# kakaobrain/rq-vae-transformer

Hardware: AMD Instinct MI355X
Metric: 256x256 images/sec, AR sampling + decode (RQ-Transformer huge, 8x8x4 codes) (higher is better)
Workload: dtype bf16

## Files before the change

### rq-vae-transformer_amd/csrc/rqt_kernels.hip

```cpp
#include "rqt_kernels.h"
#include "rq_common.h"
#include <mutex>
#include <stdlib.h>

static __device__ __forceinline__ float rq_u01(uint32_t r) { return fmaf((float)(r >> 9), 1.0f / 8388608.0f, 1.0f / 16777216.0f); }

#if defined(RQ_SAMPLE_GUIDED_TU) || defined(RQ_SAMPLE_ROWS_TU) || defined(RQ_SAMPLE_LOGP_TU)
#define RQ_SAMPLE_ONLY_TU 1
#endif
#ifndef RQ_SAMPLE_ONLY_TU

template <int NS>
__global__ __launch_bounds__(256) void resid_ln_kernel(ResidLnArgs p) {
    __shared__ float red[8];
    const int row = blockIdx.x, tid = threadIdx.x, lane = tid & 63, wave = tid >> 6;
    const int E = p.E, E4 = E >> 2;
    const long base = (long)row * E;
    const long slab_stride = (long)p.rows * E;
    f32x4 v[4];
#pragma unroll
    for (int i = 0; i < 4; ++i) {
        const int q = tid + 256 * i;
        v[i] = (f32x4){0.f, 0.f, 0.f, 0.f};
        if (q < E4) v[i] = *(const f32x4*)(p.x_in + base + q * 4);
// ... 902 lines not shown
        const int i = i0 + lane;
        const bool live = i < P;
        const int iq = live ? i : P - 1;
        float qf[64], acc[64];
#pragma unroll
        for (int c = 0; c < 8; ++c) unpack8(ld128(q0 + (long)iq * 3 * E + c * 8), qf + c * 8);
#pragma unroll
        for (int e = 0; e < 64; ++e) acc[e] = 0.f;
        float m = NEG_INF, l = 0.f;
        const int jend = i0 + 63 < P - 1 ? i0 + 63 : P - 1;
        for (int j = 0; j <= jend; ++j) {
            float dot = 0.f;
#pragma unroll
            for (int c = 0; c < 8; ++c) {
                float kf[8];
                unpack8(ld128(sK + j * 64 + c * 8), kf);
#pragma unroll
                for (int e = 0; e < 8; ++e) dot = fmaf(qf[c * 8 + e], kf[e], dot);
            }
            const float sc = j <= iq ? dot * 0.125f : NEG_INF;
            const float mn = fmaxf(m, sc);
            const float alpha = (m == NEG_INF) ? 0.f : rq_fast_exp2((m - mn) * 1.4426950408889634f);
            const float w = (sc == NEG_INF) ? 0.f : rq_fast_exp2((sc - mn) * 1.4426950408889634f);
            l = l * alpha + w;
            m = mn;
#pragma unroll
            for (int c = 0; c < 8; ++c) {
                float vf[8];
                unpack8(ld128(sV + j * 64 + c * 8), vf);
#pragma unroll
                for (int e = 0; e < 8; ++e) acc[c * 8 + e] = fmaf(w, vf[e], acc[c * 8 + e] * alpha);
            }
        }
        if (live) {
            const float inv = 1.0f / l;
            bf16_t* o = p.y + ((long)img * P + i) * E + hh * 64;
#pragma unroll
            for (int c = 0; c < 8; ++c) {
                rq_u128 u;
                u.x = pack_bf16x2(acc[c * 8 + 0] * inv, acc[c * 8 + 1] * inv); u.y = pack_bf16x2(acc[c * 8 + 2] * inv, acc[c * 8 + 3] * inv);
                u.z = pack_bf16x2(acc[c * 8 + 4] * inv, acc[c * 8 + 5] * inv); u.w = pack_bf16x2(acc[c * 8 + 6] * inv, acc[c * 8 + 7] * inv);
                st128(o + c * 8, u);
            }
        }
    }
}

#define ATTN_TILE_KEYS 64
template <bool APPEND>
__global__ __launch_bounds__(64) void attn_prefill_tiled_kernel(AttnPrefillArgs p) {
    constexpr int KT = ATTN_TILE_KEYS;
    __shared__ rq_u128 sK[KT * 8], sV[KT * 8];
    const int lane = threadIdx.x;
    const int P = p.P, E = p.E;
    const int nqt = (P + 63) / 64;
    const long blk = blockIdx.x;
    const int qt = nqt - 1 - (int)(blk % nqt);
    const long pair = blk / nqt;
    const int img = (int)(pair / p.nh), hh = (int)(pair - (long)img * p.nh);
    const bf16_t* q0 = p.qkv + (long)img * P * 3 * E + hh * 64;
    const int i0 = qt * 64, i = i0 + lane;
    const bool live = i < P;
    const int iq = live ? i : P - 1;
    const float NEG_INF = -__int_as_float(0x7f800000);
    float qf[64], acc[64];
#pragma unroll
    for (int c = 0; c < 8; ++c) unpack8(ld128(q0 + (long)iq * 3 * E + c * 8), qf + c * 8);
#pragma unroll
    for (int e = 0; e < 64; ++e) acc[e] = 0.f;
    float m = NEG_INF, l = 0.f;
    const int jend = i0 + 63 < P - 1 ? i0 + 63 : P - 1;
    for (int j0 = 0; j0 <= jend; j0 += KT) {
        const int nk = jend + 1 - j0 < KT ? jend + 1 - j0 : KT;
        rq_syncthreads();
        for (int idx = lane; idx < nk * 8; idx += 64) {
            const int j = j0 + (idx >> 3), c = idx & 7;
            const rq_u128 kv = ld128(q0 + (long)j * 3 * E + E + c * 8), vv = ld128(q0 + (long)j * 3 * E + 2 * E + c * 8);
            sK[idx] = kv;
            sV[idx] = vv;
            if (APPEND && j >= i0) {
                st128(p.kc + (pair * p.Tcap + j) * 64 + c * 8, kv);
                st128(p.vc + (pair * p.Tcap + j) * 64 + c * 8, vv);
            }
        }
        rq_syncthreads();
        for (int jj = 0; jj < nk; ++jj) {
            const int j = j0 + jj;
            float dot = 0.f;
#pragma unroll
            for (int c = 0; c < 8; ++c) {
                float kf[8];
                unpack8(sK[jj * 8 + c], kf);
#pragma unroll
                for (int e = 0; e < 8; ++e) dot = fmaf(qf[c * 8 + e], kf[e], dot);
            }
            const float sc = j <= iq ? dot * 0.125f : NEG_INF;
            const float mn = fmaxf(m, sc);
            const float alpha = (m == NEG_INF) ? 0.f : rq_fast_exp2((m - mn) * 1.4426950408889634f);
            const float w = (sc == NEG_INF) ? 0.f : rq_fast_exp2((sc - mn) * 1.4426950408889634f);
            l = l * alpha + w;
            m = mn;
#pragma unroll
            for (int c = 0; c < 8; ++c) {
                float vf[8];
                unpack8(sV[jj * 8 + c], vf);
#pragma unroll
                for (int e = 0; e < 8; ++e) acc[c * 8 + e] = fmaf(w, vf[e], acc[c * 8 + e] * alpha);
            }
        }
    }
    if (live) {
        const float inv = 1.0f / l;
        bf16_t* o = p.y + ((long)img * P + i) * E + hh * 64;
#pragma unroll
        for (int c = 0; c < 8; ++c) {
            rq_u128 u;
            u.x = pack_bf16x2(acc[c * 8 + 0] * inv, acc[c * 8 + 1] * inv); u.y = pack_bf16x2(acc[c * 8 + 2] * inv, acc[c * 8 + 3] * inv);
            u.z = pack_bf16x2(acc[c * 8 + 4] * inv, acc[c * 8 + 5] * inv); u.w = pack_bf16x2(acc[c * 8 + 6] * inv, acc[c * 8 + 7] * inv);
            st128(o + c * 8, u);
        }
    }
}

int rq_launch_attn_prefill(const AttnPrefillArgs& a, hipStream_t s) {
    const bool append = a.kc != nullptr;
    if (!append && (a.vc || a.ksc || a.vsc)) return rq_fail(RQAMD_ERR_INVALID, "prefill attention: cache-free form with a cache pointer");
    if (append && !a.vc) return rq_fail(RQAMD_ERR_INVALID, "prefill attention: key cache without a value cache");
    if (a.nh >= 1 && a.E != a.nh * 64) {
        RQ_TRY(attn_generic_check(a.E, a.nh, a.Tcap, a.ksc));
        if (a.P < 1 || a.P > a.Tcap) return rq_fail(RQAMD_ERR_UNSUPPORTED, "prefill attention: %d tokens (cache %d)", a.P, a.Tcap);
        const long blocks = (long)a.n_img * a.nh * a.P;
        if (blocks > 0x7fffffffL) return rq_fail(RQAMD_ERR_UNSUPPORTED, "prefill attention: %ld (image, head, token) triples", blocks);
        if (append) RQ_LAUNCH(attn_generic_prefill_kernel<true>, dim3((unsigned)blocks), dim3(64), 0, s, a);
        else RQ_LAUNCH(attn_generic_prefill_kernel<false>, dim3((unsigned)blocks), dim3(64), 0, s, a);
        return rq_check_launch("attn_generic_prefill_kernel");
    }
    if (a.nh < 1 || a.P < 1 || a.P > a.Tcap) return rq_fail(RQAMD_ERR_UNSUPPORTED, "prefill attention: %d tokens (cache %d)", a.P, a.Tcap);
    const char* force_tiled = getenv("RQAMD_PREFILL_TILED");
    if (a.P > 255 || (force_tiled && atoi(force_tiled) != 0 && !a.ksc)) {
        if (a.ksc || a.vsc) return rq_fail(RQAMD_ERR_UNSUPPORTED, "prefill attention: the 8-bit cache formats (RQAMD_KV) end at 255 prefix tokens (%d)", a.P);
        const long blocks = (long)a.n_img * a.nh * ((a.P + 63) / 64);
        if (blocks > 0x7fffffffL) return rq_fail(RQAMD_ERR_UNSUPPORTED, "prefill attention: %ld (image, head, query tile) triples", blocks);
        if (append) RQ_LAUNCH(attn_prefill_tiled_kernel<true>, dim3((unsigned)blocks), dim3(64), 0, s, a);
        else RQ_LAUNCH(attn_prefill_tiled_kernel<false>, dim3((unsigned)blocks), dim3(64), 0, s, a);
        return rq_check_launch("attn_prefill_tiled_kernel");
    }
    const size_t smem = (size_t)a.P * 64 * 2 * 2;
    if (append) RQ_LAUNCH(attn_prefill_kernel<true>, dim3((unsigned)(a.n_img * a.nh)), dim3(64), smem, s, a);
    else RQ_LAUNCH(attn_prefill_kernel<false>, dim3((unsigned)(a.n_img * a.nh)), dim3(64), smem, s, a);
    return rq_check_launch("attn_prefill_kernel");
}

__global__ void embed_tokens_kernel(EmbedTokArgs p) {
    const int per_row = p.dim / 8;
    const long gid = (long)blockIdx.x * blockDim.x + threadIdx.x;
    if (gid >= (long)p.rows * per_row) return;
    const int b = (int)(gid / per_row), c = (int)(gid - (long)b * per_row);
    const int pos = (p.pos ? *p.pos : 0) + p.pos_off;
    const int64_t* codes = p.xs + ((long)b * p.HW + pos) * p.D;
    float acc[8];
#pragma unroll
    for (int e = 0; e < 8; ++e) acc[e] = 0.f;
    for (int d = p.depth_lo; d < p.n_depth; ++d) {
        long code = codes[d];
        if (code < 0 || code >= p.K[d]) continue;
        const float* src = p.cb[d] + code * p.dim + c * 8;
        f32x4 a = *(const f32x4*)src, bq = *(const f32x4*)(src + 4);
#pragma unroll
        for (int e = 0; e < 4; ++e) { acc[e] += a[e]; acc[4 + e] += bq[e]; }
    }
    rq_u128 o;
    o.x = pack_bf16x2(acc[0], acc[1]); o.y = pack_bf16x2(acc[2], acc[3]);
    o.z = pack_bf16x2(acc[4], acc[5]); o.w = pack_bf16x2(acc[6], acc[7]);
    st128(p.out + (long)b * p.dim + c * 8, o);
}

int rq_launch_embed_tokens(const EmbedTokArgs& a, hipStream_t s) {
    if (a.dim % 8 != 0) return rq_fail(RQAMD_ERR_UNSUPPORTED, "embed: dim %d %% 8 != 0", a.dim);
    const long n = (long)a.rows * (a.dim / 8);
    RQ_LAUNCH(embed_tokens_kernel, dim3((unsigned)((n + 255) / 256)), dim3(256), 0, s, a);
    return rq_check_launch("embed_tokens_kernel");
}

__global__ void tok_embed_kernel(TokEmbedArgs p) {
    const int per_row = p.E / 4;
    const long gid = (long)blockIdx.x * blockDim.x + threadIdx.x;
    if (gid >= (long)p.rows * per_row) return;
    const int b = (int)(gid / per_row), c = (int)(gid - (long)b * per_row);
    const int pv = p.pos ? *p.pos : 0;
    const int64_t* codes = p.xs + ((long)b * p.HW + pv + p.pos_off) * p.D;
    const int arow = (p.add_by_pos ? pv : 0) + p.add_row;
    f32x4 acc = *(const f32x4*)(p.add + (long)arow * p.E + c * 4);
    for (int d = p.d_lo; d < p.d_hi; ++d) {
        long code = codes[d];
        if (code < 0 || code >= p.V[d]) rq_trap();
        acc = acc + *(const f32x4*)(p.table + ((long)p.offs[d] + code) * p.E + c * 4);
    }
    *(f32x4*)(p.out + (long)b * p.E + c * 4) = acc;
}
int rq_launch_tok_embed(const TokEmbedArgs& a, hipStream_t s) {
    const long n = (long)a.rows * (a.E / 4);
    RQ_LAUNCH(tok_embed_kernel, dim3((unsigned)((n + 255) / 256)), dim3(256), 0, s, a);
    return rq_check_launch("tok_embed_kernel");
}
__global__ void mask_logits_kernel(float* logits, int rows, int V, int v_lo) {
    const int w = V - v_lo;
    const long gid = (long)blockIdx.x * blockDim.x + threadIdx.x;
    if (gid >= (long)rows * w) return;
    const int r = (int)(gid / w), c = (int)(gid - (long)r * w);
    logits[(long)r * V + v_lo + c] = -__int_as_float(0x7f800000);
}
int rq_launch_mask_logits(float* logits, int rows, int V, int v_lo, hipStream_t s) {
    if (v_lo >= V) return RQAMD_OK;
    const long n = (long)rows * (V - v_lo);
    RQ_LAUNCH(mask_logits_kernel, dim3((unsigned)((n + 255) / 256)), dim3(256), 0, s, logits, rows, V, v_lo);
    return rq_check_launch("mask_logits_kernel");
}

__global__ void cond_embed_kernel(const int64_t* cond, int cond_stride, int cond_idx, const float* cond_emb, int vocab_cond,
                                  const float* pos_emb_cond, float* x, int rows, int E) {
    const long gid = (long)blockIdx.x * blockDim.x + threadIdx.x;
    if (gid >= (long)rows * E) return;
    const int b = (int)(gid / E), e = (int)(gid - (long)b * E);
    long c = cond ? cond[(long)b * cond_stride + cond_idx] : 0;
    if (c < 0) c = 0;
    if (c >= vocab_cond) c = vocab_cond - 1;
    x[gid] = cond_emb[c * E + e] + pos_emb_cond[(long)cond_idx * E + e];
}

int rq_launch_cond_embed(const int64_t* cond, int cond_stride, int cond_idx, const float* cond_emb, int vocab_cond,
                         const float* pos_emb_cond, float* x, int rows, int E, hipStream_t s) {
    const long n = (long)rows * E;
    RQ_LAUNCH(cond_embed_kernel, dim3((unsigned)((n + 255) / 256)), dim3(256), 0, s, cond, cond_stride, cond_idx,
              cond_emb, vocab_cond, pos_emb_cond, x, rows, E);
    return rq_check_launch("cond_embed_kernel");
}

__global__ void cond_embed_multi_kernel(const int64_t* cond, int cond_stride, int n_tok, const float* cond_emb, int vocab_cond,
                                        const float* pos_emb_cond, float* x, int n_img, int E) {
    const long gid = (long)blockIdx.x * blockDim.x + threadIdx.x;
    if (gid >= (long)n_img * n_tok * E) return;
    const long row = gid / E;
    const int e = (int)(gid - row * E);
    const int img = (int)(row / n_tok), i = (int)(row - (long)img * n_tok);
    long c = cond ? cond[(long)img * cond_stride + i] : 0;
    if (c < 0) c = 0;
    if (c >= vocab_cond) c = vocab_cond - 1;
    x[gid] = cond_emb[c * E + e] + pos_emb_cond[(long)i * E + e];
}

int rq_launch_cond_embed_multi(const int64_t* cond, int cond_stride, int n_tok, const float* cond_emb, int vocab_cond,
                               const float* pos_emb_cond, float* x, int n_img, int E, hipStream_t s) {
    const long n = (long)n_img * n_tok * E;
    RQ_LAUNCH(cond_embed_multi_kernel, dim3((unsigned)((n + 255) / 256)), dim3(256), 0, s, cond, cond_stride, n_tok,
              cond_emb, vocab_cond, pos_emb_cond, x, n_img, E);
    return rq_check_launch("cond_embed_multi_kernel");
}

__global__ void cvt_bf16_kernel(const float* src, bf16_t* dst, long n) {
    long i = ((long)blockIdx.x * blockDim.x + threadIdx.x) * 4;
    if (i + 3 < n) {
        f32x4 v = *(const f32x4*)(src + i);
        uint32_t lo = pack_bf16x2(v[0], v[1]), hi = pack_bf16x2(v[2], v[3]);
        *(uint32_t*)(dst + i) = lo;
        *(uint32_t*)(dst + i + 2) = hi;
    } else {
        for (; i < n; ++i) dst[i] = f32_to_bf16(src[i]);
    }
}
int rq_launch_cvt_bf16(const float* src, bf16_t* dst, long n, hipStream_t s) {
    if (n <= 0) return RQAMD_OK;
    if (((uintptr_t)src & 15) || ((uintptr_t)dst & 7)) return rq_fail(RQAMD_ERR_INVALID, "cvt_bf16: misaligned pointers");
    const long nt = (n + 3) / 4;
    RQ_LAUNCH(cvt_bf16_kernel, dim3((unsigned)((nt + 255) / 256)), dim3(256), 0, s, src, dst, n);
    return rq_check_launch("cvt_bf16_kernel");
}
__global__ void cvt_bf16_transpose_kernel(const float* src, bf16_t* dst, int R, int Cc) {
    const long gid = (long)blockIdx.x * blockDim.x + threadIdx.x;
    if (gid >= (long)R * Cc) return;
    const int c = (int)(gid / R), r = (int)(gid - (long)c * R);
    dst[gid] = f32_to_bf16(src[(long)r * Cc + c]);
}
int rq_launch_cvt_bf16_transpose(const float* src, bf16_t* dst, int R, int Cc, hipStream_t s) {
    const long n = (long)R * Cc;
    RQ_LAUNCH(cvt_bf16_transpose_kernel, dim3((unsigned)((n + 255) / 256)), dim3(256), 0, s, src, dst, R, Cc);
    return rq_check_launch("cvt_bf16_transpose_kernel");
}
__global__ void set_int_kernel(int* p, int v) { if (threadIdx.x == 0) *p = v; }
__global__ void add_int_kernel(int* p, int v) { if (threadIdx.x == 0) *p += v; }
int rq_launch_set_int(int* p, int v, hipStream_t s) {
    RQ_LAUNCH(set_int_kernel, dim3(1), dim3(64), 0, s, p, v);
    return rq_check_launch("set_int_kernel");
}
int rq_launch_add_int(int* p, int v, hipStream_t s) {
    RQ_LAUNCH(add_int_kernel, dim3(1), dim3(64), 0, s, p, v);
    return rq_check_launch("add_int_kernel");
}

#endif

#ifndef RQ_SMP_NT
#define RQ_SMP_NT 0
#endif
constexpr int SMP_T = 256;
constexpr int SMP_VPT = 64;

static __device__ __forceinline__ float blk_sum(float v, float* red) {
    const int lane = threadIdx.x & 63, wave = threadIdx.x >> 6;
    v = wave_sum(v);
    if (lane == 0) red[wave] = v;
    rq_syncthreads();
    float t = 0.f;
#pragma unroll
    for (int w = 0; w < SMP_T / 64; ++w) t += red[w];
    rq_syncthreads();
    return t;
}
static __device__ __forceinline__ float blk_sum_pp(float v, float* red2, int parity) {
    const int lane = threadIdx.x & 63, wave = threadIdx.x >> 6;
    float* red = red2 + (parity & 1) * 16;
    v = wave_sum(v);
    if (lane == 0) red[wave] = v;
    rq_syncthreads();
    float t = 0.f;
#pragma unroll
    for (int w = 0; w < SMP_T / 64; ++w) t += red[w];
    return t;
}
static __device__ __forceinline__ float blk_max(float v, float* red) {
    const int lane = threadIdx.x & 63, wave = threadIdx.x >> 6;
    v = wave_max(v);
    if (lane == 0) red[wave] = v;
    rq_syncthreads();
    float t = red[0];
#pragma unroll
    for (int w = 1; w < SMP_T / 64; ++w) t = fmaxf(t, red[w]);
    rq_syncthreads();
    return t;
}
static __device__ __forceinline__ float blk_min(float v, float* red) { return -blk_max(-v, red); }

static __device__ __forceinline__ int blk_excl_scan(int v, int* redi, int* total) {
    const int lane = threadIdx.x & 63, wave = threadIdx.x >> 6;
    int inc = v;
#pragma unroll
    for (int off = 1; off < 64; off <<= 1) {
        int o = rq_shfl_i(inc, lane >= off ? lane - off : lane);
        if (lane >= off) inc += o;
    }
    if (lane == 63) redi[wave] = inc;
    rq_syncthreads();
    int base = 0, tot = 0;
#pragma unroll
    for (int w = 0; w < SMP_T / 64; ++w) {
        if (w < wave) base += redi[w];
        tot += redi[w];
    }
    rq_syncthreads();
    *total = tot;
    return base + inc - v;
}

static __device__ __forceinline__ unsigned order_key(float f) {
    unsigned u = __float_as_uint(f);
    if ((u & 0x7fffffffu) > 0x7f800000u) return 0xffffffffu;
    if (u == 0x80000000u) u = 0u;
    return (u & 0x80000000u) ? ~u : (u | 0x80000000u);
}

static __device__ __forceinline__ void philox4x32_10(unsigned c0, unsigned c1, unsigned c2, unsigned c3,
                                                     unsigned k0, unsigned k1, unsigned* out) {
#pragma unroll
    for (int r = 0; r < 10; ++r) {
        const unsigned hi0 = __umulhi(0xD2511F53u, c0), lo0 = 0xD2511F53u * c0;
        const unsigned hi1 = __umulhi(0xCD9E8D57u, c2), lo1 = 0xCD9E8D57u * c2;
        const unsigned n0 = hi1 ^ c1 ^ k0, n1 = lo1, n2 = hi0 ^ c3 ^ k1, n3 = lo0;
        c0 = n0; c1 = n1; c2 = n2; c3 = n3;
        k0 += 0x9E3779B9u; k1 += 0xBB67AE85u;
    }
    out[0] = c0; out[1] = c1; out[2] = c2; out[3] = c3;
}

static __device__ __forceinline__ bool sample_kept(const SampleArgs& p, int row) {
    return p.keep && p.keep[(long)row * p.keep_stride + (p.pos ? (*p.pos) * p.D + p.d : 0)] != 0;
}

static __device__ __forceinline__ float guide_logit(float c, float u, float s) {
    return c == -__int_as_float(0x7f800000) ? c : fmaf(s - 1.0f, c - u, c);
}

enum { SMP_ROW_GUMBEL = 0, SMP_ROW_TOPK = 1, SMP_ROW_GENERAL = 2 };
static __device__ __forceinline__ int sample_row_class(const SampleArgs& p, int row) {
    const int k = p.row_top_k[(long)row * p.D + p.d];
    const float tp = p.row_top_p[(long)row * p.D + p.d];
    const bool k_on = k > 0 && k < p.V;
    if (!k_on && (tp < 0.f || tp >= 1.0f) && !p.probs_out && p.out) return SMP_ROW_GUMBEL;
    if (k_on && p.V <= SMP_T * SMP_VPT && p.V % 4 == 0 && p.redo) return SMP_ROW_TOPK;
    return SMP_ROW_GENERAL;
}
static __device__ __forceinline__ void sample_row_params(SampleArgs& p, int row) {
    p.temperature = p.row_temperature[row];
    p.top_k = p.row_top_k[(long)row * p.D + p.d];
    p.top_p = p.row_top_p[(long)row * p.D + p.d];
    if (p.row_gscale) p.gscale = p.row_gscale[row];
    if (p.row_seeds) { p.rng = nullptr; p.seed = p.row_seeds[row]; }
}

template <bool GUIDED>
static __device__ __forceinline__ void sample_store(const SampleArgs& p, int row, int slot, int code) {
    const long o = (long)row * p.out_stride + slot;
    p.out[o] = (int64_t)code;
    if (GUIDED && p.out_mirror) p.out[o + p.out_mirror] = (int64_t)code;
}

template <bool GUIDED, bool ROWS = false, bool LOGP = false>
__global__ __launch_bounds__(256) void sample_kernel(SampleArgs p) {
    RQ_DYN_SMEM(smem);
    float* sx = (float*)smem;
    float* red = sx + p.V;
    int* redi = (int*)(red + 16);
    float* red2 = (float*)(redi + 16) + 256 + 4;
    unsigned* hist = (unsigned*)(redi + 16);
    unsigned* bcast = hist + 256;
    const int tid = threadIdx.x, V = p.V, row = blockIdx.x;
    if (sample_kept(p, row)) return;
    if (ROWS) {
        const int cls = sample_row_class(p, row);
        if (cls == SMP_ROW_GUMBEL || (cls == SMP_ROW_TOPK && !p.redo[row])) return;
        sample_row_params(p, row);
    }
    if (!ROWS && p.redo && !p.redo[row]) return;
    const int prow = (ROWS && p.row_seeds) ? 0 : row;
    const float* lg = p.logits + (long)row * V;
    const float NEG_INF = -__int_as_float(0x7f800000);

    if (GUIDED) {
        const float* lu = p.logits_u + (long)row * V;
        for (int i = tid; i < V; i += SMP_T) sx[i] = guide_logit(lg[i], lu[i], p.gscale) / p.temperature;
    } else {
        for (int i = tid; i < V; i += SMP_T) sx[i] = lg[i] / p.temperature;
    }
    rq_syncthreads();

    if (p.top_k > 0 && p.top_k < V) {
        unsigned prefix = 0;
        int remaining = p.top_k;
        for (int pass = 3; pass >= 0; --pass) {
            for (int i = tid; i < 256; i += SMP_T) hist[i] = 0;
            rq_syncthreads();
            const int shift = pass * 8;
            for (int i = tid; i < V; i += SMP_T) {
                const unsigned k = order_key(sx[i]);
                if (pass == 3 || (k >> (shift + 8)) == prefix) atomicAdd(&hist[(k >> shift) & 255u], 1u);
            }
            rq_syncthreads();
            const int bin = 255 - tid;
            const int cnt = (tid < 256) ? (int)hist[bin] : 0;
            int total;
            const int excl = blk_excl_scan(cnt, redi, &total);
            if (tid < 256 && excl < remaining && excl + cnt >= remaining) { bcast[0] = (unsigned)bin; bcast[1] = (unsigned)(remaining - excl); }
            rq_syncthreads();
            prefix = (prefix << 8) | bcast[0];
            remaining = (int)bcast[1];
            rq_syncthreads();
        }
        if (prefix != 0xffffffffu)
            for (int i = tid; i < V; i += SMP_T)
                if (order_key(sx[i]) < prefix) sx[i] = NEG_INF;
        rq_syncthreads();
    }

    float mx = NEG_INF;
    for (int i = tid; i < V; i += SMP_T) {
        float v = sx[i];
        if (v != v) { v = NEG_INF; sx[i] = v; }
        mx = fmaxf(mx, v);
    }
    mx = blk_max(mx, red);
    float z = 0.f;
    for (int i = tid; i < V; i += SMP_T) {
        const float e = expf(sx[i] - mx);
        sx[i] = e;
        z += e;
    }
    z = blk_sum(z, red);
    for (int i = tid; i < V; i += SMP_T) sx[i] = sx[i] / z;
    rq_syncthreads();

    if (p.top_p >= 0.f && p.top_p < 1.0f) {
        const float top_p = fmaxf(p.top_p, 1.17549435e-38f);
        unsigned cur = 0;
        const bool in_regs = V <= SMP_T * SMP_VPT;
        float pv[SMP_VPT];
#pragma unroll
        for (int k = 0; k < SMP_VPT; ++k) {
            const int i = tid + k * SMP_T;
            pv[k] = (in_regs && i < V) ? sx[i] : 0.f;
        }
        for (int bit = 30; bit >= 0; --bit) {
            const unsigned cand = cur | (1u << bit);
            const float cv = __uint_as_float(cand);
            if (cand > 0x3f800000u) continue;
            float g = 0.f;
            if (in_regs) {
                float g0 = 0.f, g1 = 0.f, g2 = 0.f, g3 = 0.f;
#pragma unroll
                for (int k = 0; k < SMP_VPT; k += 4) {
                    g0 += pv[k] >= cv ? pv[k] : 0.f;
                    g1 += pv[k + 1] >= cv ? pv[k + 1] : 0.f;
                    g2 += pv[k + 2] >= cv ? pv[k + 2] : 0.f;
                    g3 += pv[k + 3] >= cv ? pv[k + 3] : 0.f;
                }
                g = (g0 + g1) + (g2 + g3);
            } else {
                for (int i = tid; i < V; i += SMP_T) { const float q = sx[i]; if (q >= cv) g += q; }
            }
            g = blk_sum_pp(g, red2, bit);
            if (g >= top_p) cur = cand;
        }
        const float tau = __uint_as_float(cur);
        float vmin = 2.0f;
        for (int i = tid; i < V; i += SMP_T) { const float q = sx[i]; if (q >= tau) vmin = fminf(vmin, q); }
        vmin = blk_min(vmin, red);
        float gs = 0.f;
        int nt = 0;
        const int per = (V + SMP_T - 1) / SMP_T, i0 = tid * per, i1 = (i0 + per < V) ? i0 + per : V;
        for (int i = i0; i < i1; ++i) { const float q = sx[i]; if (q > vmin) gs += q; else if (q == vmin) ++nt; }
        gs = blk_sum(gs, red);
        int ntie;
        int rank = blk_excl_scan(nt, redi, &ntie);
        int need = ntie;
        if (vmin > 0.f) {
            float m = ceilf((top_p - gs) / vmin);
            if (m < 1.f) m = 1.f;
            if (m < (float)ntie) need = (int)m;
        }
        float kept = 0.f;
        for (int i = i0; i < i1; ++i) {
            float q = sx[i];
            if (q < vmin) q = 0.f;
            else if (q == vmin) { if (rank >= need) q = 0.f; ++rank; }
            sx[i] = q;
            kept += q;
        }
        kept = blk_sum(kept, red);
        for (int i = tid; i < V; i += SMP_T) sx[i] = sx[i] / kept;
        rq_syncthreads();
    }

    if (p.probs_out)
        for (int i = tid; i < V; i += SMP_T) p.probs_out[(long)row * V + i] = sx[i];
    if (!p.out) return;

    const int slot = p.pos ? (*p.pos) * p.D + p.d : 0;
    const uint64_t seed = p.rng ? p.rng[0] : p.seed;
    const uint64_t off = (p.rng ? p.rng[1] : p.offset) + (uint64_t)slot;
    float best = -1.f;
    int besti = 0x7fffffff;
    for (int i4 = tid; i4 * 4 < V; i4 += SMP_T) {
        unsigned r[4];
        philox4x32_10((unsigned)i4, (unsigned)prow, (unsigned)off, (unsigned)(off >> 32), (unsigned)seed, (unsigned)(seed >> 32), r);
#pragma unroll
        for (int e = 0; e < 4; ++e) {
            const int i = i4 * 4 + e;
            if (i < V) {
                const float u = rq_u01(r[e]);
                const float sc = sx[i] / (-logf(u));
                if (sc > best) { best = sc; besti = i; }
            }
        }
    }
    const int lane = tid & 63, wave = tid >> 6;
#pragma unroll
    for (int m = 32; m >= 1; m >>= 1) {
        const float ov = rq_shfl_xor(best, m);
        const int oi = rq_shfl_xor_i(besti, m);
        if (ov > best || (ov == best && oi < besti)) { best = ov; besti = oi; }
    }
    if (lane == 0) { red[wave] = best; redi[wave] = besti; }
    rq_syncthreads();
    if (tid == 0) {
        for (int w = 1; w < SMP_T / 64; ++w)
            if (red[w] > best || (red[w] == best && redi[w] < besti)) { best = red[w]; besti = redi[w]; }
        if (besti >= V) besti = 0;
        sample_store<GUIDED>(p, row, slot, besti);
        if (LOGP) p.logp_out[(long)row * p.out_stride + slot] = logf(sx[besti]);
    }
}

constexpr int SMP_CAP = 2048;
constexpr int SMP_CV = SMP_CAP / SMP_T;
constexpr int SMP_UND = 256;

static __device__ __forceinline__ float key_to_float(unsigned k) {
    return __uint_as_float((k & 0x80000000u) ? (k ^ 0x80000000u) : ~k);
}

struct SmpShared {
    float red[16];
    int redi[16];
    float red2[32];
    int cnt[2][4];
    unsigned bc[4];
    unsigned und[SMP_UND];
    int und_n;
    float val[SMP_CAP];
    int idx[SMP_CAP];
};

static __device__ __forceinline__ int blk_count_pp(int wave_cnt, SmpShared& sh, int parity) {
    const int lane = threadIdx.x & 63, wave = threadIdx.x >> 6;
    if (lane == 0) sh.cnt[parity & 1][wave] = wave_cnt;
    rq_syncthreads();
    return (sh.cnt[parity & 1][0] + sh.cnt[parity & 1][1]) + (sh.cnt[parity & 1][2] + sh.cnt[parity & 1][3]);
}

template <bool GUIDED, bool ROWS, bool LOGP, int NV, typename IdxF>
static __device__ __forceinline__ void sample_tail(const SampleArgs& p, float (&q)[NV], IdxF idx_of, int row, SmpShared& sh) {
    const int tid = threadIdx.x, V = p.V;
    const float NEG_INF = -__int_as_float(0x7f800000);
    float mx = NEG_INF;
#pragma unroll
    for (int k = 0; k < NV; ++k) {
        float v = idx_of(k) >= 0 ? q[k] : NEG_INF;
        if (v != v) v = NEG_INF;
        q[k] = v;
        mx = fmaxf(mx, v);
    }
    mx = blk_max(mx, sh.red);
    float z = 0.f;
#pragma unroll
    for (int k = 0; k < NV; ++k) {
        const float e = idx_of(k) >= 0 ? expf(q[k] - mx) : 0.f;
        q[k] = e;
        z += e;
    }
    z = blk_sum(z, sh.red);
#pragma unroll
    for (int k = 0; k < NV; ++k) q[k] = q[k] / z;

    if (p.top_p >= 0.f && p.top_p < 1.0f) {
        const float top_p = fmaxf(p.top_p, 1.17549435e-38f);
        unsigned cur = 0;
        for (int bit = 30; bit >= 0; --bit) {
            const unsigned cand = cur | (1u << bit);
            const float cv = __uint_as_float(cand);
            if (cand > 0x3f800000u) continue;
            float g0 = 0.f, g1 = 0.f, g2 = 0.f, g3 = 0.f;
#pragma unroll
            for (int k = 0; k < NV; k += 4) {
                g0 += q[k] >= cv ? q[k] : 0.f;
                g1 += q[k + 1] >= cv ? q[k + 1] : 0.f;
                g2 += q[k + 2] >= cv ? q[k + 2] : 0.f;
                g3 += q[k + 3] >= cv ? q[k + 3] : 0.f;
            }
            const float g = blk_sum_pp((g0 + g1) + (g2 + g3), sh.red2, bit);
            if (g >= top_p) cur = cand;
        }
        const float tau = __uint_as_float(cur);
        float vmin = 2.0f;
#pragma unroll
        for (int k = 0; k < NV; ++k) if (q[k] >= tau) vmin = fminf(vmin, q[k]);
        vmin = blk_min(vmin, sh.red);
        float gs = 0.f;
        int nt = 0;
#pragma unroll
        for (int k = 0; k < NV; ++k) { if (q[k] > vmin) gs += q[k]; else if (q[k] == vmin && idx_of(k) >= 0) ++nt; }
        gs = blk_sum(gs, sh.red);
        int ntie;
        (void)blk_excl_scan(nt, sh.redi, &ntie);
        int need = ntie;
        if (vmin > 0.f) {
            float m = ceilf((top_p - gs) / vmin);
            if (m < 1.f) m = 1.f;
            if (m < (float)ntie) need = (int)m;
        }
        int cut = 0x7fffffff;
        if (need < ntie) {
            unsigned ci = 0;
            for (int bit = 14; bit >= 0; --bit) {
                const unsigned cand = ci | (1u << bit);
                int c = 0;
#pragma unroll
                for (int k = 0; k < NV; ++k) c += (q[k] == vmin && idx_of(k) >= 0 && (unsigned)idx_of(k) < cand) ? 1 : 0;
                c = wave_sum_i(c);
                if (blk_count_pp(c, sh, bit) < need) ci = cand;
            }
            cut = (int)ci;
        }
        float kept = 0.f;
#pragma unroll
        for (int k = 0; k < NV; ++k) {
            float v = q[k];
            if (v < vmin || (v == vmin && idx_of(k) > cut)) v = 0.f;
            q[k] = v;
            kept += v;
        }
        kept = blk_sum(kept, sh.red);
#pragma unroll
        for (int k = 0; k < NV; ++k) q[k] = q[k] / kept;
    }

    if (p.probs_out) {
#pragma unroll
        for (int k = 0; k < NV; ++k)
            if (idx_of(k) >= 0) p.probs_out[(long)row * V + idx_of(k)] = q[k];
    }
    if (!p.out) return;

    const int slot = p.pos ? (*p.pos) * p.D + p.d : 0;
    const uint64_t seed = p.rng ? p.rng[0] : p.seed;
    const uint64_t off = (p.rng ? p.rng[1] : p.offset) + (uint64_t)slot;
    const int prow = (ROWS && p.row_seeds) ? 0 : row;
    float best = -1.f;
    int besti = 0x7fffffff;
    float bestq = 0.f;
#pragma unroll
    for (int k = 0; k < NV; ++k) {
        const int i = idx_of(k);
        if (i < 0) continue;
        unsigned r[4];
        philox4x32_10((unsigned)(i >> 2), (unsigned)prow, (unsigned)off, (unsigned)(off >> 32), (unsigned)seed, (unsigned)(seed >> 32), r);
        const unsigned w = (i & 3) == 0 ? r[0] : (i & 3) == 1 ? r[1] : (i & 3) == 2 ? r[2] : r[3];
        const float u = rq_u01(w);
        const float sc = q[k] / (-logf(u));
        if (sc > best || (sc == best && i < besti)) { best = sc; besti = i; if (LOGP) bestq = q[k]; }
    }
    const int lane = tid & 63, wave = tid >> 6;
#pragma unroll
    for (int m = 32; m >= 1; m >>= 1) {
        const float ov = rq_shfl_xor(best, m);
        const int oi = rq_shfl_xor_i(besti, m);
        const float oq = LOGP ? rq_shfl_xor(bestq, m) : 0.f;
        if (ov > best || (ov == best && oi < besti)) { best = ov; besti = oi; if (LOGP) bestq = oq; }
    }
    if (lane == 0) { sh.red[wave] = best; sh.redi[wave] = besti; if (LOGP) sh.red2[wave] = bestq; }
    rq_syncthreads();
    if (tid == 0) {
        for (int w = 1; w < SMP_T / 64; ++w)
            if (sh.red[w] > best || (sh.red[w] == best && sh.redi[w] < besti)) { best = sh.red[w]; besti = sh.redi[w]; if (LOGP) bestq = sh.red2[w]; }
        if (besti >= V) besti = 0;
        sample_store<GUIDED>(p, row, slot, besti);
        if (LOGP) p.logp_out[(long)row * p.out_stride + slot] = logf(bestq);
    }
}

template <bool GUIDED, bool ROWS = false, bool LOGP = false>
__global__ __launch_bounds__(SMP_T) void sample_topk_kernel(SampleArgs p) {
    __shared__ SmpShared sh;
    const int tid = threadIdx.x, lane = tid & 63, V = p.V, row = blockIdx.x;
    if (sample_kept(p, row)) return;
    if (ROWS) {
        if (sample_row_class(p, row) != SMP_ROW_TOPK) return;
        sample_row_params(p, row);
    }
    const float* lg = p.logits + (long)row * V;
    const int V4 = V >> 2;
    unsigned ks[SMP_VPT];
    const bool scale = p.temperature != 1.0f;
#pragma unroll
    for (int j = 0; j < SMP_VPT / 4; ++j) {
        const int i4 = tid + SMP_T * j;
#if RQ_SMP_NT
        f32x4 v = __builtin_nontemporal_load((const f32x4*)(lg + (long)(i4 < V4 ? i4 : V4 - 1) * 4));
#else
        f32x4 v = *(const f32x4*)(lg + (long)(i4 < V4 ? i4 : V4 - 1) * 4);
#endif
        if (GUIDED) {
            const float* lu = p.logits_u + (long)row * V;
#if RQ_SMP_NT
            const f32x4 vu = __builtin_nontemporal_load((const f32x4*)(lu + (long)(i4 < V4 ? i4 : V4 - 1) * 4));
#else
            const f32x4 vu = *(const f32x4*)(lu + (long)(i4 < V4 ? i4 : V4 - 1) * 4);
#endif
#pragma unroll
            for (int e = 0; e < 4; ++e) v[e] = guide_logit(v[e], vu[e], p.gscale);
        }
#pragma unroll
        for (int e = 0; e < 4; ++e) {
            const float x = scale ? v[e] / p.temperature : v[e];
            ks[4 * j + e] = i4 < V4 ? order_key(x) : 0u;
        }
    }

    unsigned kth = 0;
    {
        unsigned cur = 0;
        for (int bit = 31; bit >= 16; --bit) {
            const unsigned cand = cur | (1u << bit);
            int c = 0;
#pragma unroll
            for (int k = 0; k < SMP_VPT; ++k) c += ks[k] >= cand ? 1 : 0;
            if (blk_count_pp(wave_sum_i(c), sh, bit) >= p.top_k) cur = cand;
        }
        if (tid == 0) sh.und_n = 0;
        rq_syncthreads();
        const unsigned pre = cur >> 16;
        int above = 0;
#pragma unroll
        for (int k = 0; k < SMP_VPT; ++k) {
            above += (ks[k] >> 16) > pre ? 1 : 0;
            if ((ks[k] >> 16) == pre) {
                const int pos = atomicAdd(&sh.und_n, 1);
                if (pos < SMP_UND) sh.und[pos] = ks[k];
            }
        }
        above = blk_count_pp(wave_sum_i(above), sh, 0);
        const int und_n = sh.und_n;
        const int need = p.top_k - above;
        if (und_n <= SMP_UND) {
            if (tid < 64) {
                unsigned uk[SMP_UND / 64];
#pragma unroll
                for (int m = 0; m < SMP_UND / 64; ++m) uk[m] = (lane + 64 * m < und_n) ? sh.und[lane + 64 * m] : 0u;
                for (int bit = 15; bit >= 0; --bit) {
                    const unsigned cand = cur | (1u << bit);
                    int c = 0;
#pragma unroll
                    for (int m = 0; m < SMP_UND / 64; ++m) c += rq_popc64(rq_ballot(uk[m] >= cand));
                    if (c >= need) cur = cand;
                }
                if (lane == 0) sh.bc[0] = cur;
            }
            rq_syncthreads();
            cur = sh.bc[0];
        } else {
            for (int bit = 15; bit >= 0; --bit) {
                const unsigned cand = cur | (1u << bit);
                int c = 0;
#pragma unroll
                for (int k = 0; k < SMP_VPT; ++k) c += ks[k] >= cand ? 1 : 0;
                if (blk_count_pp(wave_sum_i(c), sh, bit) >= p.top_k) cur = cand;
            }
        }
        kth = cur;
    }
    const bool cutk = kth != 0xffffffffu;
    int mine = 0;
#pragma unroll
    for (int k = 0; k < SMP_VPT; ++k) mine += ks[k] >= kth ? 1 : 0;
    int total = 0;
    const int base = blk_excl_scan(mine, sh.redi, &total);
    const bool compact = cutk && total <= SMP_CAP;
    if (tid == 0) p.redo[row] = compact ? 0 : 1;
    if (!compact) return;

    int pos = base;
#pragma unroll
    for (int k = 0; k < SMP_VPT; ++k)
        if (ks[k] >= kth) { sh.val[pos] = key_to_float(ks[k]); sh.idx[pos] = (tid + SMP_T * (k >> 2)) * 4 + (k & 3); ++pos; }
    if (p.probs_out) {
#pragma unroll
        for (int j = 0; j < SMP_VPT / 4; ++j)
            if (tid + SMP_T * j < V4) *(f32x4*)(p.probs_out + (long)row * V + (tid + SMP_T * j) * 4) = (f32x4){0.f, 0.f, 0.f, 0.f};
        rq_threadfence_block();
    }
    rq_syncthreads();
    float q[SMP_CV];
    int qi[SMP_CV];
#pragma unroll
    for (int k = 0; k < SMP_CV; ++k) {
        const int s = tid + SMP_T * k;
        q[k] = s < total ? sh.val[s] : 0.f;
        qi[k] = s < total ? sh.idx[s] : -1;
    }
    rq_syncthreads();
    sample_tail<GUIDED, ROWS, LOGP, SMP_CV>(p, q, [&](int k) -> int { return qi[k]; }, row, sh);
}

template <bool GUIDED, bool ROWS = false, bool LOGP = false>
__global__ __launch_bounds__(256) void sample_gumbel_kernel(SampleArgs p) {
    __shared__ float red[4];
    __shared__ int redi[4];
    __shared__ float redx[LOGP ? 4 : 1];
    const int tid = threadIdx.x, V = p.V, row = blockIdx.x;
    if (sample_kept(p, row)) return;
    if (ROWS) {
        if (sample_row_class(p, row) != SMP_ROW_GUMBEL) return;
        sample_row_params(p, row);
    }
    const int prow = (ROWS && p.row_seeds) ? 0 : row;
    const float* lg = p.logits + (long)row * V;
    const float inv_t = 1.0f / p.temperature;
    const int slot = p.pos ? (*p.pos) * p.D + p.d : 0;
    const uint64_t seed = p.rng ? p.rng[0] : p.seed;
    const uint64_t off = (p.rng ? p.rng[1] : p.offset) + (uint64_t)slot;
    const float NEG_INF = -__int_as_float(0x7f800000);
    float best = NEG_INF;
    int besti = 0x7fffffff;
    float bestx = NEG_INF, lm = NEG_INF, lsum = 0.f;
    const bool vec = (V & 3) == 0;
    for (int i4 = tid; i4 * 4 < V; i4 += 256) {
        float v[4];
        if (vec) {
            const f32x4 q = *(const f32x4*)(lg + i4 * 4);
            v[0] = q[0]; v[1] = q[1]; v[2] = q[2]; v[3] = q[3];
        } else {
#pragma unroll
            for (int e = 0; e < 4; ++e) v[e] = (i4 * 4 + e < V) ? lg[i4 * 4 + e] : NEG_INF;
        }
        if (GUIDED) {
            const float* lu = p.logits_u + (long)row * V;
            float w[4];
            if (vec) {
                const f32x4 q = *(const f32x4*)(lu + i4 * 4);
                w[0] = q[0]; w[1] = q[1]; w[2] = q[2]; w[3] = q[3];
            } else {
#pragma unroll
                for (int e = 0; e < 4; ++e) w[e] = (i4 * 4 + e < V) ? lu[i4 * 4 + e] : NEG_INF;
            }
#pragma unroll
            for (int e = 0; e < 4; ++e) v[e] = guide_logit(v[e], w[e], p.gscale);
        }
        unsigned r[4];
        philox4x32_10((unsigned)i4, (unsigned)prow, (unsigned)off, (unsigned)(off >> 32), (unsigned)seed, (unsigned)(seed >> 32), r);
#pragma unroll
        for (int e = 0; e < 4; ++e) {
            const int i = i4 * 4 + e;
            const float u = rq_u01(r[e]);
            float x = v[e] * inv_t;
            if (x != x) x = NEG_INF;
            const float sc = x - __logf(-__logf(u));
            if (i < V && sc > best) { best = sc; besti = i; if (LOGP) bestx = x; }
            if (LOGP && i < V) {
                if (x > lm) { lsum = lsum * expf(lm - x) + 1.0f; lm = x; }
                else if (!(x <= NEG_INF)) lsum += expf(x - lm);
            }
        }
    }
    float M = 0.f, S = 0.f;
    if (LOGP) {
        M = blk_max(lm, red);
        S = blk_sum(lm > NEG_INF ? lsum * expf(lm - M) : 0.f, red);
    }
    const int lane = tid & 63, wave = tid >> 6;
#pragma unroll
    for (int m = 32; m >= 1; m >>= 1) {
        const float ov = rq_shfl_xor(best, m);
        const int oi = rq_shfl_xor_i(besti, m);
        const float ox = LOGP ? rq_shfl_xor(bestx, m) : 0.f;
        if (ov > best || (ov == best && oi < besti)) { best = ov; besti = oi; if (LOGP) bestx = ox; }
    }
    if (lane == 0) { red[wave] = best; redi[wave] = besti; if (LOGP) redx[wave] = bestx; }
    rq_syncthreads();
    if (tid == 0) {
        for (int w = 1; w < 4; ++w)
            if (red[w] > best || (red[w] == best && redi[w] < besti)) { best = red[w]; besti = redi[w]; if (LOGP) bestx = redx[w]; }
        if (besti >= V) besti = 0;
        sample_store<GUIDED>(p, row, slot, besti);
        if (LOGP) p.logp_out[(long)row * p.out_stride + slot] = (bestx - M) - logf(S);
    }
}

template <bool GUIDED, bool LOGP = false>
static int launch_sample(const SampleArgs& a, hipStream_t s) {
    if (a.V < 1 || a.V > 36000) return rq_fail(RQAMD_ERR_UNSUPPORTED, "sampler: vocab %d not in 1..36000", a.V);
    if (!(a.temperature > 0.f)) return rq_fail(RQAMD_ERR_INVALID, "sampler: temperature must be > 0");
    if (GUIDED && !(a.gscale - a.gscale == 0.f)) return rq_fail(RQAMD_ERR_INVALID, "sampler: guidance scale must be finite");
    if ((a.top_k <= 0 || a.top_k >= a.V) && (a.top_p < 0.f || a.top_p >= 1.0f) && !a.probs_out && a.out) {
        const auto kern = sample_gumbel_kernel<GUIDED, false, LOGP>;
        RQ_LAUNCH(kern, dim3(a.rows), dim3(256), 0, s, a);
        return rq_check_launch("sample_gumbel_kernel");
    }
    const size_t smem = (size_t)a.V * 4 + 16 * 4 + 16 * 4 + 256 * 4 + 4 * 4 + 32 * 4;
    static RqDeviceOnce attr_once;
    if (attr_once.first()) {
        (void)hipFuncSetAttribute((const void*)sample_kernel<GUIDED, false, LOGP>, hipFuncAttributeMaxDynamicSharedMemorySize, 160 * 1024);
    }
    SampleArgs b = a;
    static const bool env_lds_only = getenv("RQAMD_SAMPLER_LDS") != nullptr;
    if (a.top_k > 0 && a.top_k < a.V && a.V <= SMP_T * SMP_VPT && a.V % 4 == 0 && a.redo && !env_lds_only) {
        const auto kern = sample_topk_kernel<GUIDED, false, LOGP>;
        RQ_LAUNCH(kern, dim3(a.rows), dim3(SMP_T), 0, s, a);
        RQ_TRY(rq_check_launch("sample_topk_kernel"));
    } else {
        b.redo = nullptr;
    }
    const auto gen = sample_kernel<GUIDED, false, LOGP>;
    RQ_LAUNCH(gen, dim3(a.rows), dim3(SMP_T), smem, s, b);
    return rq_check_launch("sample_kernel");
}

#if defined(RQ_SAMPLE_ROWS_TU) || defined(RQ_SAMPLE_LOGP_TU)
template <bool GUIDED, bool LOGP = false>
static int launch_sample_per_row(const SampleArgs& a, hipStream_t s) {
    if (a.V < 1 || a.V > 36000) return rq_fail(RQAMD_ERR_UNSUPPORTED, "sampler: vocab %d not in 1..36000", a.V);
    if (!a.row_top_k || !a.row_top_p) return rq_fail(RQAMD_ERR_INVALID, "sampler: per-row top_k / top_p missing");
    SampleArgs b = a;
    static const bool env_lds_only = getenv("RQAMD_SAMPLER_LDS") != nullptr;
    if (env_lds_only) b.redo = nullptr;
    if (!b.probs_out && b.out) {
        const auto kern = sample_gumbel_kernel<GUIDED, true, LOGP>;
        RQ_LAUNCH(kern, dim3(b.rows), dim3(256), 0, s, b);
        RQ_TRY(rq_check_launch("sample_gumbel_kernel (per row)"));
    }
    if (b.V <= SMP_T * SMP_VPT && b.V % 4 == 0 && b.redo) {
        const auto kern = sample_topk_kernel<GUIDED, true, LOGP>;
        RQ_LAUNCH(kern, dim3(b.rows), dim3(SMP_T), 0, s, b);
        RQ_TRY(rq_check_launch("sample_topk_kernel (per row)"));
    }
    const size_t smem = (size_t)b.V * 4 + 16 * 4 + 16 * 4 + 256 * 4 + 4 * 4 + 32 * 4;
    const auto kern = sample_kernel<GUIDED, true, LOGP>;
    static RqDeviceOnce attr_once;
    if (attr_once.first()) {
        (void)hipFuncSetAttribute((const void*)kern, hipFuncAttributeMaxDynamicSharedMemorySize, 160 * 1024);
    }
    RQ_LAUNCH(kern, dim3(b.rows), dim3(SMP_T), smem, s, b);
    return rq_check_launch("sample_kernel (per row)");
}
#endif
#ifdef RQ_SAMPLE_ROWS_TU
int rq_launch_sample_per_row(const SampleArgs& a, hipStream_t s) {
    return a.logits_u ? launch_sample_per_row<true>(a, s) : launch_sample_per_row<false>(a, s);
}
#elif defined(RQ_SAMPLE_LOGP_TU)
int rq_launch_sample_logp(const SampleArgs& a, hipStream_t s) {
    if (a.row_temperature) return a.logits_u ? launch_sample_per_row<true, true>(a, s) : launch_sample_per_row<false, true>(a, s);
    return a.logits_u ? launch_sample<true, true>(a, s) : launch_sample<false, true>(a, s);
}
#elif defined(RQ_SAMPLE_GUIDED_TU)
int rq_launch_sample_guided(const SampleArgs& a, hipStream_t s) { return launch_sample<true>(a, s); }
#else
int rq_launch_sample_guided(const SampleArgs& a, hipStream_t s);
int rq_launch_sample_per_row(const SampleArgs& a, hipStream_t s);
int rq_launch_sample_logp(const SampleArgs& a, hipStream_t s);
int rq_launch_sample(const SampleArgs& a, hipStream_t s) {
    if (a.logp_out) return rq_launch_sample_logp(a, s);
    if (a.row_temperature) return rq_launch_sample_per_row(a, s);
    return a.logits_u ? rq_launch_sample_guided(a, s) : launch_sample<false>(a, s);
}

__global__ __launch_bounds__(256) void guide_logits_kernel(const float* c, const float* u, float* out, long n, int vec, float s) {
    const long i = (long)blockIdx.x * 256 + threadIdx.x;
    if (vec) {
        if (i * 4 >= n) return;
        const f32x4 a = *(const f32x4*)(c + i * 4), b = *(const f32x4*)(u + i * 4);
        f32x4 g;
#pragma unroll
        for (int e = 0; e < 4; ++e) g[e] = guide_logit(a[e], b[e], s);
        *(f32x4*)(out + i * 4) = g;
    } else {
        if (i >= n) return;
        out[i] = guide_logit(c[i], u[i], s);
    }
}
int rq_launch_guide_logits(const float* c, const float* u, int rows, int V, float scale, float* out, hipStream_t s) {
    if (!c || !u || !out || rows < 0 || V < 1) return rq_fail(RQAMD_ERR_INVALID, "guide_logits: bad argument");
    if (!(scale - scale == 0.f)) return rq_fail(RQAMD_ERR_INVALID, "guide_logits: scale must be finite");
    if (rows == 0) return RQAMD_OK;
    const long n = (long)rows * V;
    const int vec = V % 4 == 0 && (((uintptr_t)c | (uintptr_t)u | (uintptr_t)out) & 15) == 0;
    const long nt = vec ? n / 4 : n;
    RQ_LAUNCH(guide_logits_kernel, dim3((unsigned)((nt + 255) / 256)), dim3(256), 0, s, c, u, out, n, vec, scale);
    return rq_check_launch("guide_logits_kernel");
}
extern "C" int rqamd_guide_logits(const float* cond_logits, const float* uncond_logits, int rows, int vocab, float scale, float* out, void* stream) {
    return rq_launch_guide_logits(cond_logits, uncond_logits, rows, vocab, scale, out, (hipStream_t)stream);
}

int rq_launch_sample_rows(const float* logits, int rows, int vocab, uint64_t seed, uint64_t offset, int64_t* out, long out_stride, hipStream_t s) {
    SampleArgs a{};
    a.logits = logits; a.rows = rows; a.V = vocab; a.temperature = 1.0f; a.top_k = 0; a.top_p = -1.0f;
    a.seed = seed; a.offset = offset; a.out = out; a.out_stride = out_stride; a.D = 1;
    return rq_launch_sample(a, s);
}

extern "C" int rqamd_sample_logits(const float* logits, int rows, int vocab, float temperature, int top_k, float top_p,
                                   uint64_t seed, uint64_t offset, int64_t* samples_out, float* probs_out, int* row_flags, void* stream) {
    if (!logits || rows < 0) return rq_fail(RQAMD_ERR_INVALID, "sample_logits: bad argument");
    if (rows == 0) return RQAMD_OK;
    SampleArgs a{};
    a.logits = logits; a.rows = rows; a.V = vocab; a.temperature = temperature; a.top_k = top_k; a.top_p = top_p;
    a.seed = seed; a.offset = offset; a.out = samples_out; a.out_stride = 1; a.probs_out = probs_out; a.D = 1;
    a.redo = row_flags;
    return rq_launch_sample(a, (hipStream_t)stream);
}

extern "C" int rqamd_sample_logits_rows(const float* logits, int rows, int vocab, const float* temperature, const int* top_k,
                                        const float* top_p, const uint64_t* seeds, uint64_t seed, uint64_t offset,
                                        int64_t* samples_out, float* probs_out, int* row_flags, void* stream) {
    if (!logits || rows < 0 || !temperature || !top_k || !top_p) return rq_fail(RQAMD_ERR_INVALID, "sample_logits_rows: bad argument (null array or rows < 0)");
    if (rows == 0) return RQAMD_OK;
    SampleArgs a{};
    a.logits = logits; a.rows = rows; a.V = vocab; a.temperature = 1.0f; a.top_k = 0; a.top_p = -1.0f;
    a.seed = seed; a.offset = offset; a.out = samples_out; a.out_stride = 1; a.probs_out = probs_out; a.D = 1;
    a.redo = row_flags;
    a.row_temperature = temperature; a.row_top_k = top_k; a.row_top_p = top_p; a.row_seeds = seeds;
    return rq_launch_sample(a, (hipStream_t)stream);
}
// ... 424 lines not shown
```

Before: 1623.

## Find top-k threshold with a value-range histogram before radix fallback

Replaces the 16-pass bitwise radix select in the top-k sampling kernel with a single-pass histogram. It bins logits over their min-max range into 2048 shared-memory bins, finds the bin that holds the k-th element with a block scan, and resolves that bin exactly with a one-wave bitwise select. This is meant to cut the many block-wide count and sync rounds per row. It falls back to the old radix path when the range is degenerate or the boundary bin overflows the candidate buffer, and it adds shared atomics that can contend on skewed distributions.

New measurement: 1626 (median of 4 runs). Within noise of the previous version (+0.2%).

```diff
diff --git a/rq-vae-transformer_amd/csrc/rqt_kernels.hip b/rq-vae-transformer_amd/csrc/rqt_kernels.hip
--- a/rq-vae-transformer_amd/csrc/rqt_kernels.hip
+++ b/rq-vae-transformer_amd/csrc/rqt_kernels.hip
@@ -1228,6 +1228,9 @@
 #ifndef RQ_SMP_NT
 #define RQ_SMP_NT 0
 #endif
+#ifndef RQ_SMP_HIST
+#define RQ_SMP_HIST 1
+#endif
 constexpr int SMP_T = 256;
 constexpr int SMP_VPT = 64;
 
@@ -1541,6 +1544,29 @@
     return (sh.cnt[parity & 1][0] + sh.cnt[parity & 1][1]) + (sh.cnt[parity & 1][2] + sh.cnt[parity & 1][3]);
 }
 
+constexpr int SMP_NB = 2048;
+static_assert(SMP_NB * sizeof(unsigned) <= sizeof(float) * SMP_CAP && SMP_NB % SMP_T == 0, "the bins live in SmpShared::val, a whole number per thread");
+static __device__ __forceinline__ int smp_bin(float x, float lo, float s) {
+    const int b = (int)((x - lo) * s);
+    return b < SMP_NB - 1 ? b : SMP_NB - 1;
+}
+static __device__ __forceinline__ void blk_minmax_u(unsigned& lo, unsigned& hi, int* redi) {
+    const int lane = threadIdx.x & 63, wave = threadIdx.x >> 6;
+#pragma unroll
+    for (int m = 32; m >= 1; m >>= 1) {
+        const unsigned ol = (unsigned)rq_shfl_xor_i((int)lo, m), oh = (unsigned)rq_shfl_xor_i((int)hi, m);
+        lo = ol < lo ? ol : lo;
+        hi = oh > hi ? oh : hi;
+    }
+    if (lane == 0) { redi[wave] = (int)lo; redi[4 + wave] = (int)hi; }
+    rq_syncthreads();
+#pragma unroll
+    for (int w = 0; w < SMP_T / 64; ++w) {
+        lo = (unsigned)redi[w] < lo ? (unsigned)redi[w] : lo;
+        hi = (unsigned)redi[4 + w] > hi ? (unsigned)redi[4 + w] : hi;
+    }
+}
+
 template <bool GUIDED, bool ROWS, bool LOGP, int NV, typename IdxF>
 static __device__ __forceinline__ void sample_tail(const SampleArgs& p, float (&q)[NV], IdxF idx_of, int row, SmpShared& sh) {
     const int tid = threadIdx.x, V = p.V;
@@ -1683,6 +1709,9 @@
     const float* lg = p.logits + (long)row * V;
     const int V4 = V >> 2;
     unsigned ks[SMP_VPT];
+#if RQ_SMP_HIST
+    unsigned kmin = 0xffffffffu, kmax = 0u;
+#endif
     const bool scale = p.temperature != 1.0f;
 #pragma unroll
     for (int j = 0; j < SMP_VPT / 4; ++j) {
@@ -1706,11 +1735,78 @@
         for (int e = 0; e < 4; ++e) {
             const float x = scale ? v[e] / p.temperature : v[e];
             ks[4 * j + e] = i4 < V4 ? order_key(x) : 0u;
+#if RQ_SMP_HIST
+            kmax = ks[4 * j + e] > kmax ? ks[4 * j + e] : kmax;
+            kmin = (i4 < V4 && ks[4 * j + e] < kmin) ? ks[4 * j + e] : kmin;
+#endif
         }
     }
 
     unsigned kth = 0;
+    bool settled = false;
+#if RQ_SMP_HIST
     {
+        unsigned* hist = (unsigned*)sh.val;
+#pragma unroll
+        for (int b = 0; b < SMP_NB / SMP_T; ++b) hist[SMP_NB - 1 - (SMP_NB / SMP_T) * tid - b] = 0u;
+        if (tid == 0) sh.und_n = 0;
+        unsigned klo = kmin, khi = kmax;
+        blk_minmax_u(klo, khi, sh.redi);
+        const float lo = key_to_float(klo), hi = key_to_float(khi);
+        const float s = (float)SMP_NB / (hi - lo);
+        const float INF = __int_as_float(0x7f800000);
+        if (fabsf(lo) < INF && fabsf(hi) < INF && hi > lo && (hi - lo) < INF && s < INF) {
+#pragma unroll
+            for (int k = 0; k < SMP_VPT; ++k)
+                if (tid + SMP_T * (k >> 2) < V4) atomicAdd(&hist[smp_bin(key_to_float(ks[k]), lo, s)], 1u);
+            rq_syncthreads();
+            unsigned h[SMP_NB / SMP_T];
+            int cnt = 0;
+#pragma unroll
+            for (int b = 0; b < SMP_NB / SMP_T; ++b) { h[b] = hist[SMP_NB - 1 - (SMP_NB / SMP_T) * tid - b]; cnt += (int)h[b]; }
+            int nkeys = 0;
+            int acc = blk_excl_scan(cnt, sh.redi, &nkeys);
+            if (acc < p.top_k && acc + cnt >= p.top_k) {
+#pragma unroll
+                for (int b = 0; b < SMP_NB / SMP_T; ++b) {
+                    if (acc < p.top_k && acc + (int)h[b] >= p.top_k) { sh.bc[1] = (unsigned)(SMP_NB - 1 - (SMP_NB / SMP_T) * tid - b); sh.bc[2] = (unsigned)acc; }
+                    acc += (int)h[b];
+                }
+            }
+            rq_syncthreads();
+            const int bstar = (int)sh.bc[1];
+            const int need = p.top_k - (int)sh.bc[2];
+#pragma unroll
+            for (int k = 0; k < SMP_VPT; ++k)
+                if (tid + SMP_T * (k >> 2) < V4 && smp_bin(key_to_float(ks[k]), lo, s) == bstar) {
+                    const int pos = atomicAdd(&sh.und_n, 1);
+                    if (pos < SMP_UND) sh.und[pos] = ks[k];
+                }
+            rq_syncthreads();
+            const int und_n = sh.und_n;
+            if (und_n <= SMP_UND) {
+                if (tid < 64) {
+                    unsigned uk[SMP_UND / 64];
+#pragma unroll
+                    for (int m = 0; m < SMP_UND / 64; ++m) uk[m] = (lane + 64 * m < und_n) ? sh.und[lane + 64 * m] : 0u;
+                    unsigned cur = 0;
+                    for (int bit = 31; bit >= 0; --bit) {
+                        const unsigned cand = cur | (1u << bit);
+                        int c = 0;
+#pragma unroll
+                        for (int m = 0; m < SMP_UND / 64; ++m) c += rq_popc64(rq_ballot(uk[m] >= cand));
+                        if (c >= need) cur = cand;
+                    }
+                    if (lane == 0) sh.bc[0] = cur;
+                }
+                rq_syncthreads();
+                kth = sh.bc[0];
+                settled = true;
+            }
+        }
+    }
+#endif
+    if (!settled) {
         unsigned cur = 0;
         for (int bit = 31; bit >= 16; --bit) {
             const unsigned cand = cur | (1u << bit);
```
